# windingwind/seal-3d

Hardware: AMD Instinct MI355X
Metric: train samples/s (NGP -O step on synthetic Lego 800x800 rays) (higher is better)
Workload: dtype f16; 1 GPU; configs[1]: nerf_synthetic/lego-shaped NGP -O (hashgrid L16 F2 T2^19 + ffmlp 64x2/64x3 + raymarching), 800x800 cameras, 4096 rays/step/GPU; num_rays_per_gpu=4096, parallelism=ray-sharded dp1, pretrain_steps=384, launch=hip-graph replay

## Files before the change

### seal-3d_amd/csrc/raymarching.hip

```cpp
#include "s3d_common.hpp"
#include "s3d_step_tail.hpp"

namespace s3d {
namespace {

constexpr float kSqrt3 = 1.7320508075688772f;
constexpr float kRPi = 0.3183098861837907f;

__device__ __forceinline__ uint32_t expand_bits_any(uint32_t v) {
    v = (v * 0x00010001u) & 0xFF0000FFu;
    v = (v * 0x00000101u) & 0x0F00F00Fu;
    v = (v * 0x00000011u) & 0xC30C30C3u;
    v = (v * 0x00000005u) & 0x49249249u;
    return v;
}
__device__ __forceinline__ uint32_t expand_bits(uint32_t v) {
    v = (v | (v << 16)) & 0xFF0000FFu;
    v = (v | (v << 8)) & 0x0F00F00Fu;
    v = (v | (v << 4)) & 0xC30C30C3u;
    v = (v | (v << 2)) & 0x49249249u;
    return v;
}
__device__ __forceinline__ uint32_t morton3d(uint32_t x, uint32_t y, uint32_t z) {
    return expand_bits(x) | (expand_bits(y) << 1) | (expand_bits(z) << 2);
// ... 353 lines not shown
        const float s = sweep_sum_partials(partial + (size_t)c * stride, nblocks, wsum);
        total = c == 0 ? s : total + s;
    }
    if (threadIdx.x == 0) {
        const float mean = total * inv_n;
        record->mean = mean;
        record->thresh = density_thresh < mean ? density_thresh : mean;
        int32_t rows = *local_step;
        rows = rows < 0 ? 0 : (rows > 16 ? 16 : rows);
        int64_t count = 0;
        for (int32_t r = 0; r < rows; r++) count += step_ring[2 * r];
        record->count_lo = (uint32_t)((uint64_t)count & 0xFFFFFFFFull);
        record->count_hi = (uint32_t)((uint64_t)count >> 32);
        if (sweep_step) *sweep_step += 1;
    }
}

struct Ray {
    float ox, oy, oz, dx, dy, dz, rdx, rdy, rdz;
};
struct MarchParams {
    float bound, dt_gamma, dt_min, dt_max, rH, H3, Cf, Hf, Hm1, halfH;
    const uint8_t* grid;
};

__device__ __forceinline__ MarchParams make_params(float bound, float dt_gamma, uint32_t max_steps, uint32_t C,
                                                   uint32_t H, const uint8_t* grid) {
    MarchParams p;
    p.bound = bound; p.dt_gamma = dt_gamma;
    p.dt_min = 2 * kSqrt3 / (float)max_steps;
    p.dt_max = 2 * kSqrt3 * (float)(1 << (C - 1)) / (float)H;
    p.rH = 1 / (float)H;
    p.H3 = (float)(H * H * H);
    p.Cf = (float)C; p.Hf = (float)H; p.Hm1 = (float)(H - 1); p.halfH = 0.5f * (float)H;
    p.grid = grid;
    return p;
}

__device__ __forceinline__ Ray load_ray(const float* __restrict__ rays_o, const float* __restrict__ rays_d, uint32_t n) {
    Ray r;
    r.ox = rays_o[n * 3]; r.oy = rays_o[n * 3 + 1]; r.oz = rays_o[n * 3 + 2];
    r.dx = rays_d[n * 3]; r.dy = rays_d[n * 3 + 1]; r.dz = rays_d[n * 3 + 2];
    r.rdx = 1 / r.dx; r.rdy = 1 / r.dy; r.rdz = 1 / r.dz;
    return r;
}

__device__ __forceinline__ int mip_from_pos(float x, float y, float z, float Cf) {
    int e;
    (void)frexpf(fmaxf(fabsf(x), fmaxf(fabsf(y), fabsf(z))), &e);
    return (int)fminf(Cf - 1, fmaxf(0.0f, (float)e));
}
__device__ __forceinline__ int mip_from_dt(float dt, float Hf, float Cf) {
    int e;
    (void)frexpf((dt * Hf) * 0.5f, &e);
    return (int)fminf(Cf - 1, fmaxf(0.0f, (float)e));
}
__device__ __forceinline__ int mip_level(float x, float y, float z, float dt, const MarchParams& p) {
    const int la = mip_from_pos(x, y, z, p.Cf), lb = mip_from_dt(dt, p.Hf, p.Cf);
    return la > lb ? la : lb;
}

__global__ void k_mip_levels(const float* __restrict__ xyz, const float* __restrict__ dt, uint32_t N, float Hf, float Cf,
                             int32_t* __restrict__ mip_pos, int32_t* __restrict__ mip_dt) {
    for (uint32_t n = blockIdx.x * blockDim.x + threadIdx.x; n < N; n += gridDim.x * blockDim.x) {
        if (mip_pos) mip_pos[n] = mip_from_pos(xyz[n * 3], xyz[n * 3 + 1], xyz[n * 3 + 2], Cf);
        if (mip_dt) mip_dt[n] = mip_from_dt(dt[n], Hf, Cf);
    }
}

struct ProbeCell {
    float x, y, z, dt, mip_bound;
    int nx, ny, nz;
};
__device__ __forceinline__ uint32_t probe_cell(const Ray& r, const MarchParams& p, float t, ProbeCell& c) {
    c.x = clampf(__builtin_fmaf(t, r.dx, r.ox), -p.bound, p.bound);
    c.y = clampf(__builtin_fmaf(t, r.dy, r.oy), -p.bound, p.bound);
    c.z = clampf(__builtin_fmaf(t, r.dz, r.oz), -p.bound, p.bound);
    c.dt = clampf(t * p.dt_gamma, p.dt_min, p.dt_max);
    const int level = mip_level(c.x, c.y, c.z, c.dt, p);
    c.mip_bound = fminf(ldexpf(1.0f, level), p.bound);
    const float mip_rbound = 1 / c.mip_bound;
    c.nx = (int)clampf(__builtin_fmaf(c.x, mip_rbound, 1.0f) * p.halfH, 0.0f, p.Hm1);
    c.ny = (int)clampf(__builtin_fmaf(c.y, mip_rbound, 1.0f) * p.halfH, 0.0f, p.Hm1);
    c.nz = (int)clampf(__builtin_fmaf(c.z, mip_rbound, 1.0f) * p.halfH, 0.0f, p.Hm1);
    return (uint32_t)((float)level * p.H3 + (float)morton3d((uint32_t)c.nx, (uint32_t)c.ny, (uint32_t)c.nz));
}
__device__ __forceinline__ float probe_exit(const Ray& r, const MarchParams& p, float t, const ProbeCell& c) {
    const float sx = copysignf(1.0f, r.dx), sy = copysignf(1.0f, r.dy), sz = copysignf(1.0f, r.dz);
    const float tx = __builtin_fmaf(__builtin_fmaf(__builtin_fmaf(0.5f, sx, (float)c.nx + 0.5f) * p.rH, 2.0f, -1.0f), c.mip_bound, -c.x) * r.rdx;
    const float ty = __builtin_fmaf(__builtin_fmaf(__builtin_fmaf(0.5f, sy, (float)c.ny + 0.5f) * p.rH, 2.0f, -1.0f), c.mip_bound, -c.y) * r.rdy;
    const float tz = __builtin_fmaf(__builtin_fmaf(__builtin_fmaf(0.5f, sz, (float)c.nz + 0.5f) * p.rH, 2.0f, -1.0f), c.mip_bound, -c.z) * r.rdz;
    return t + fmaxf(0.0f, fminf(tx, fminf(ty, tz)));
}
__device__ __forceinline__ bool probe(const Ray& r, const MarchParams& p, float t, float& x, float& y, float& z,
                                      float& dt, float& t_skip) {
    ProbeCell c;
    const uint32_t index = probe_cell(r, p, t, c);
    x = c.x; y = c.y; z = c.z; dt = c.dt;
    const bool occ = (p.grid[index >> 3] & (1u << (index & 7u))) != 0;
    if (!occ) t_skip = probe_exit(r, p, t, c);
    return occ;
}

__device__ __forceinline__ float skip_to(const MarchParams& p, float t, float tt) {
    do { t += clampf(t * p.dt_gamma, p.dt_min, p.dt_max); } while (t < tt);
    return t;
}

constexpr uint32_t kWsHeader = 4;

__global__ void __launch_bounds__(64) k_march_count(const float* __restrict__ rays_o, const float* __restrict__ rays_d,
                                                    const uint8_t* __restrict__ grid, float bound, float dt_gamma,
                                                    uint32_t max_steps, uint32_t N, uint32_t C, uint32_t H,
                                                    const float* __restrict__ nears, const float* __restrict__ fars,
                                                    const float* __restrict__ noises, int32_t* __restrict__ rays,
                                                    const int32_t* __restrict__ counter, uint32_t* __restrict__ ws) {
    const uint32_t n = blockIdx.x * 64 + threadIdx.x;
    uint32_t num_steps = 0;
    if (n < N) {
        const MarchParams p = make_params(bound, dt_gamma, max_steps, C, H, grid);
        const Ray r = load_ray(rays_o, rays_d, n);
        const float far = fars[n];
        float t = nears[n];
        t = __builtin_fmaf(clampf(t * dt_gamma, p.dt_min, p.dt_max), noises[n], t);
        while (t < far && num_steps < max_steps) {
            float x, y, z, dt, tt;
            if (probe(r, p, t, x, y, z, dt, tt)) { num_steps++; t += dt; }
            else t = skip_to(p, t, tt);
        }
    }
    const uint32_t incl = wave_incl_scan(num_steps);
    if (n < N) {
        rays[n * 3] = (int32_t)n;
        rays[n * 3 + 1] = (int32_t)(incl - num_steps);
        rays[n * 3 + 2] = (int32_t)num_steps;
    }
    if (threadIdx.x == 63) ws[kWsHeader + blockIdx.x] = incl;
    if (blockIdx.x == 0 && threadIdx.x == 0) ws[0] = (uint32_t)counter[0];
}

__global__ void __launch_bounds__(64) k_march_write(const float* __restrict__ rays_o, const float* __restrict__ rays_d,
                                                    const uint8_t* __restrict__ grid, float bound, float dt_gamma,
                                                    uint32_t max_steps, uint32_t N, uint32_t C, uint32_t H, uint32_t M,
                                                    const float* __restrict__ nears, const float* __restrict__ fars,
                                                    const float* __restrict__ noises, float* __restrict__ xyzs,
                                                    float* __restrict__ dirs, float* __restrict__ deltas,
                                                    int32_t* __restrict__ rays, int32_t* __restrict__ counter,
                                                    const uint32_t* __restrict__ ws) {
    uint32_t part = 0;
    for (uint32_t i = threadIdx.x; i < blockIdx.x; i += 64) part += ws[kWsHeader + i];
#pragma unroll
    for (int d = 32; d >= 1; d >>= 1) part += __shfl_xor(part, d, 64);
    const uint32_t base = ws[0] + part;
    if (blockIdx.x == gridDim.x - 1 && threadIdx.x == 0) {
        counter[0] = (int32_t)(base + ws[kWsHeader + blockIdx.x]);
        counter[1] = counter[1] + (int32_t)N;
    }
    const uint32_t n = blockIdx.x * 64 + threadIdx.x;
    if (n >= N) return;
    const uint32_t num_steps = (uint32_t)rays[n * 3 + 2];
    const uint32_t off = base + (uint32_t)rays[n * 3 + 1];
    rays[n * 3 + 1] = (int32_t)off;
    if (n == N - 1 && off + num_steps < M) zero_sample_rows(xyzs, dirs, deltas, off + num_steps, pad_end(off + num_steps, M), 0, 1);
    if (num_steps != 0 && off < M && off + num_steps > M) zero_sample_rows(xyzs, dirs, deltas, off, M, 0, 1);
    if (num_steps == 0 || off + num_steps > M) return;

    const MarchParams p = make_params(bound, dt_gamma, max_steps, C, H, grid);
    const Ray r = load_ray(rays_o, rays_d, n);
    const float far = fars[n];
    float t = nears[n];
    t = __builtin_fmaf(clampf(t * dt_gamma, p.dt_min, p.dt_max), noises[n], t);
    float last_t = t;
    float* px = xyzs + (size_t)off * 3;
    float* pd = dirs + (size_t)off * 3;
    float* pl = deltas + (size_t)off * 2;
    uint32_t step = 0;
    while (t < far && step < num_steps) {
        float x, y, z, dt, tt;
        if (probe(r, p, t, x, y, z, dt, tt)) {
            px[0] = x; px[1] = y; px[2] = z;
            pd[0] = r.dx; pd[1] = r.dy; pd[2] = r.dz;
            t += dt;
            pl[0] = dt; pl[1] = t - last_t;
            last_t = t;
            px += 3; pd += 3; pl += 2; step++;
        } else t = skip_to(p, t, tt);
    }
}


constexpr uint32_t kWin = 1024;
constexpr uint16_t kOcc = 0xFFFF;

template <bool CONST_DT, bool FAST>
__global__ void __launch_bounds__(64) __attribute__((amdgpu_waves_per_eu(4, 4))) k_march_count_wave(const float* __restrict__ rays_o, const float* __restrict__ rays_d,
                                                         const uint8_t* __restrict__ grid, float bound, float dt_gamma,
                                                         uint32_t max_steps, uint32_t N, uint32_t C, uint32_t H,
                                                         float* __restrict__ nears, float* __restrict__ fars,
                                                         float* __restrict__ noises, int32_t* __restrict__ rays,
                                                         const int32_t* __restrict__ counter, uint32_t* __restrict__ ws,
                                                         const float* __restrict__ aabb, float min_near,
                                                         const int32_t* __restrict__ noise_step, uint32_t noise_key) {
    __shared__ float T[kWin + 8];
    __shared__ uint16_t J[2][kWin + 2];
    __shared__ uint32_t mk[64];
    __shared__ uint32_t s_wn;
    __shared__ uint32_t lut[FAST ? 128 : 1];
    const uint32_t n = blockIdx.x, lane = threadIdx.x;
    if constexpr (FAST) {
        lut[lane] = expand_bits(lane);
        lut[lane + 64] = expand_bits(lane + 64);
    }
    const MarchParams p = make_params(bound, dt_gamma, max_steps, C, H, grid);
    const Ray r = load_ray(rays_o, rays_d, n);
    float far, t_carry, noise;
    if (aabb) {
        const float a[6] = {aabb[0], aabb[1], aabb[2], aabb[3], aabb[4], aabb[5]};
        near_far_of(rays_o, rays_d, n, a, min_near, t_carry, far);
        noise = noises ? (noise_step ? ray_noise(noise_key, (uint32_t)*noise_step, n) : noises[n]) : 0.0f;
        if (lane == 0) {
            nears[n] = t_carry;
            fars[n] = far;
            if (noises && noise_step) noises[n] = noise;
        }
    } else {
        far = fars[n];
        t_carry = nears[n];
        noise = noises[n];
    }
    const float dt0 = clampf(0.0f, p.dt_min, p.dt_max);
    auto dtf = [&](float t) { return CONST_DT ? dt0 : clampf(t * dt_gamma, p.dt_min, p.dt_max); };
    t_carry = __builtin_fmaf(clampf(t_carry * dt_gamma, p.dt_min, p.dt_max), noise, t_carry);
    float* tout = reinterpret_cast<float*>(ws + kWsHeader + N) + (size_t)n * max_steps;

    uint32_t num_steps = 0;
    float pending_tt = -INFINITY;
#ifdef S3D_MARCH_PROFILE
    long long tp[5] = {0, 0, 0, 0, 0};
    long long c0 = wall_clock64();
#define S3D_TICK(i) { const long long c1 = wall_clock64(); tp[i] += c1 - c0; c0 = c1; }
#else
#define S3D_TICK(i)
#endif
    for (;;) {
        if constexpr (CONST_DT) {
            float t = t_carry;
            uint32_t k = 0;
            const uint32_t bfar = __float_as_uint(far);
            while (k < kWin && t < far) {
                const float t1 = t + dt0, t2 = t1 + dt0;
                const uint32_t b0 = __float_as_uint(t), b1 = __float_as_uint(t1), b2 = __float_as_uint(t2);
                const uint32_t inc = b2 - b1;
                if (!(t > 0.0f) || (b0 >> 23) != (b2 >> 23) || (b0 >> 23) == 0 || inc == 0 || !(far > 0.0f) || bfar >= 0x7f800000u) {
                    if (lane == 0) T[k] = t;
                    k++;
                    t = t1;
                    continue;
                }
                const uint32_t hi = ((b1 >> 23) + 1) << 23;
                const uint32_t cnt = (hi - b1) / inc + 1;
                const uint32_t nfill = min(cnt, kWin - k);
                const uint32_t n_lt = bfar <= b1 ? 0u : min(cnt, (bfar - b1 + inc - 1) / inc);
                if (lane == 0) T[k] = t;
                for (uint32_t j = lane; j < nfill; j += 64) T[k + 1 + j] = __uint_as_float(b1 + j * inc);
                if (n_lt < nfill) {
                    k = k + 1 + n_lt;
                    t = __uint_as_float(b1 + n_lt * inc);
                    break;
                }
                k += nfill;
                t = __uint_as_float(b1 + (nfill - 1) * inc);
            }
            if (lane == 0) { T[k] = t; s_wn = k; }
        } else if (lane == 0) {
            float t = t_carry;
            uint32_t k = 0;
            while (k < kWin && t < far) {
                float v[8];
                v[0] = t;
#pragma unroll
                for (uint32_t i = 1; i < 8; i++) v[i] = v[i - 1] + dtf(v[i - 1]);
#pragma unroll
                for (uint32_t i = 0; i < 8; i++) T[k + i] = v[i];
                uint32_t c = 1;
#pragma unroll
                for (uint32_t i = 1; i < 8; i++) c += (v[i] < far) ? 1u : 0u;
                if (c < 8) {
                    float tn = v[1];
#pragma unroll
                    for (uint32_t i = 2; i < 8; i++) tn = (c == i) ? v[i] : tn;
                    k += c;
                    t = tn;
                    break;
                }
                k += 8;
                t = v[7] + dtf(v[7]);
            }
            T[k] = t;
            s_wn = k;
        }
        __syncthreads();
        S3D_TICK(0)
        const uint32_t wn = s_wn;
        uint32_t occm = 0;
        uint32_t headm = 0;
        auto skip_index = [&](uint32_t k, float tk, float tt) {
            const float t1 = T[k + 1];
            const float est = (tt - t1) / fmaxf(t1 - tk, 1e-30f);
            uint32_t m = k + 1 + (est > 0.0f ? (est < (float)kWin ? (uint32_t)est : kWin) : 0u);
            m = m < wn ? m : wn;
            while (m > k + 1 && !(T[m - 1] < tt)) m--;
            while (m < wn && T[m] < tt) m++;
            return (uint16_t)m;
        };
        if constexpr (FAST) {
            constexpr uint32_t kBatch = 8;
            const float mip_bound = fminf(1.0f, p.bound), mip_rbound = 1 / mip_bound;
            uint32_t prev_last = 0xffffffffu;
#pragma unroll 1
            for (uint32_t b0 = 0; b0 * 64 < wn; b0 += kBatch) {
                uint32_t bits[kBatch], idx[kBatch], cell[kBatch];
#pragma unroll
                for (uint32_t j = 0; j < kBatch; j++) {
                    const float t = T[lane + 64 * (b0 + j)];
                    const float x = clampf(__builtin_fmaf(t, r.dx, r.ox), -p.bound, p.bound);
                    const float y = clampf(__builtin_fmaf(t, r.dy, r.oy), -p.bound, p.bound);
                    const float z = clampf(__builtin_fmaf(t, r.dz, r.oz), -p.bound, p.bound);
                    const uint32_t nx = (uint32_t)(int)clampf(__builtin_fmaf(x, mip_rbound, 1.0f) * p.halfH, 0.0f, p.Hm1);
                    const uint32_t ny = (uint32_t)(int)clampf(__builtin_fmaf(y, mip_rbound, 1.0f) * p.halfH, 0.0f, p.Hm1);
                    const uint32_t nz = (uint32_t)(int)clampf(__builtin_fmaf(z, mip_rbound, 1.0f) * p.halfH, 0.0f, p.Hm1);
                    cell[j] = nx | (ny << 8) | (nz << 16);
                    idx[j] = (uint32_t)(float)(lut[nx] | (lut[ny] << 1) | (lut[nz] << 2));
                }
#pragma unroll
                for (uint32_t j = 0; j < kBatch; j++) bits[j] = (uint32_t)p.grid[idx[j] >> 3];
#pragma unroll
                for (uint32_t j = 0; j < kBatch; j++) {
                    const uint32_t i = b0 + j, k = lane + 64 * i;
                    uint32_t prev = (uint32_t)__builtin_amdgcn_update_dpp((int)cell[j], (int)cell[j], 0x138, 0xF, 0xF, false);
                    if (lane == 0) prev = prev_last;
                    prev_last = (uint32_t)__builtin_amdgcn_readlane((int)cell[j], 63);
                    if (cell[j] != prev) headm |= 1u << i;
                    if (k < wn) {
                        uint16_t e = (uint16_t)(k + 1);
                        if (bits[j] & (1u << (idx[j] & 7u))) {
                            occm |= 1u << i;
                        } else {
                            const float tk = T[k];
                            ProbeCell c;
                            c.x = clampf(__builtin_fmaf(tk, r.dx, r.ox), -p.bound, p.bound);
                            c.y = clampf(__builtin_fmaf(tk, r.dy, r.oy), -p.bound, p.bound);
                            c.z = clampf(__builtin_fmaf(tk, r.dz, r.oz), -p.bound, p.bound);
                            c.mip_bound = mip_bound;
                            c.nx = (int)(cell[j] & 255u); c.ny = (int)((cell[j] >> 8) & 255u); c.nz = (int)(cell[j] >> 16);
                            e = skip_index(k, tk, probe_exit(r, p, tk, c));
                        }
                        J[0][k] = e;
                    }
                }
            }
        } else {
            for (uint32_t k = lane; k < wn; k += 64) {
                float x, y, z, dt, tt;
                uint16_t e = (uint16_t)(k + 1);
                const float tk = T[k];
                if (!probe(r, p, tk, x, y, z, dt, tt)) e = skip_index(k, tk, tt);
                else occm |= 1u << (k >> 6);
                J[0][k] = e;
            }
        }
        S3D_TICK(1)
        if (lane == 0) J[0][wn] = (uint16_t)wn;
        mk[lane] = 0;
        uint32_t start = wn;
        for (uint32_t k = lane; k < wn; k += 64)
            if (!(T[k] < pending_tt)) { start = k; break; }
#pragma unroll
        for (int d = 32; d >= 1; d >>= 1) start = min(start, (uint32_t)__shfl_xor((int)start, d, 64));
        pending_tt = -INFINITY;
        __syncthreads();
        bool marked = false;
#ifdef S3D_MARCH_PROFILE
        uint32_t dbg_vm0 = 0;
#endif
        if constexpr (FAST) {
            uint32_t vm = 0;
#pragma unroll
            for (uint32_t i = 0; i < kWin / 64; i++) {
                const uint32_t k = lane + 64 * i;
                const bool in = k < wn && k >= start;
                if (in && ((((occm | headm) >> i) & 1u) || k == start)) vm |= 1u << i;
            }
            const uint32_t startbit = (start < wn && (start & 63u) == lane) ? (1u << (start >> 6)) : 0u;
#ifdef S3D_MARCH_PROFILE
            dbg_vm0 = vm;
#endif
            constexpr uint32_t kMaxPasses = 6;
            for (uint32_t pass = 0; pass < kMaxPasses && !marked; pass++) {
#pragma unroll
                for (uint32_t i = 0; i < kWin / 64; i++) {
                    if ((vm >> i) & 1u) {
                        const uint32_t tg = J[0][lane + 64 * i];
                        if (tg < wn) atomicOr(&mk[tg & 63], 1u << (tg >> 6));
                    }
                }
                __syncthreads();
                const uint32_t pm = mk[lane];
                const bool closed = __ballot((pm & ~vm) != 0u) == 0ull;
                const bool supported = __ballot((vm & ~startbit & ~pm) != 0u) == 0ull;
                marked = closed && supported;
                if (!marked) vm = closed ? (pm | startbit) : (vm | pm);
                __syncthreads();
                mk[lane] = marked ? vm : 0u;
                __syncthreads();
            }
        }
        if (!marked && lane == 0 && start < wn) mk[start & 63] = 1u << (start >> 6);
        __syncthreads();
        uint32_t cur = 0;
        constexpr uint32_t kPer = kWin / 64 + 1;
        const uint32_t iters = wn / 64 + 1;
        for (uint32_t span = 1; span < wn && !marked; span <<= 1) {
            const uint16_t* Jc = J[cur];
            uint16_t* Jn = J[cur ^ 1];
            uint32_t j1[kPer], j2[kPer];
            const uint32_t mw = mk[lane];
#pragma unroll
            for (uint32_t i = 0; i < kPer; i++)
                if (i < iters) { const uint32_t k = lane + 64 * i; j1[i] = k <= wn ? Jc[k] : wn; }
#pragma unroll
            for (uint32_t i = 0; i < kPer; i++)
                if (i < iters) j2[i] = Jc[j1[i]];
#pragma unroll
            for (uint32_t i = 0; i < kPer; i++)
                if (i < iters) {
                    const uint32_t k = lane + 64 * i;
                    if (((mw >> i) & 1u) && j1[i] < wn) atomicOr(&mk[j1[i] & 63], 1u << (j1[i] >> 6));
                    if (k <= wn) Jn[k] = (uint16_t)j2[i];
                }
            cur ^= 1;
            __syncthreads();
            if (start >= wn || J[cur][start] >= wn) break;
        }
        S3D_TICK(2)
#ifdef S3D_MARCH_PROFILE
        if (FAST && max_steps >= 256) {
            const uint32_t d = mk[lane] ^ dbg_vm0;
            uint32_t cnt = __popc(d), first = d ? (lane + 64u * (uint32_t)__builtin_ctz(d)) : 0xFFFFu;
#pragma unroll
            for (int s2 = 32; s2 >= 1; s2 >>= 1) { cnt += (uint32_t)__shfl_xor((int)cnt, s2, 64); first = min(first, (uint32_t)__shfl_xor((int)first, s2, 64)); }
            if (lane == 0) { tout[max_steps - 16] = (float)cnt; tout[max_steps - 15] = (float)first; tout[max_steps - 14] = (float)wn; tout[max_steps - 13] = (float)start; }
        }
#endif
        uint32_t last_empty = kWin;
        bool any_empty = false;
        for (uint32_t k0 = 0; k0 < wn && num_steps < max_steps; k0 += 64) {
            const uint32_t k = k0 + lane;
            const bool vis = k < wn && ((mk[lane] >> (k0 >> 6)) & 1u);
            const bool emit = vis && ((occm >> (k0 >> 6)) & 1u);
            if (vis && !emit) { last_empty = k; any_empty = true; }
            const unsigned long long m = __ballot(emit);
            const uint32_t rank = __builtin_amdgcn_mbcnt_hi((uint32_t)(m >> 32), __builtin_amdgcn_mbcnt_lo((uint32_t)m, 0u));
            if (emit && num_steps + rank < max_steps) tout[num_steps + rank] = T[k];
            num_steps = min(max_steps, num_steps + (uint32_t)__popcll(m));
        }
        uint32_t le = any_empty ? last_empty : 0u;
#pragma unroll
        for (int d = 32; d >= 1; d >>= 1) le = max(le, (uint32_t)__shfl_xor((int)le, d, 64));
        const bool had_empty = __ballot(any_empty) != 0;
        const bool more = (wn == kWin) && (num_steps < max_steps);
        if (more && had_empty) {
            float x, y, z, dt, tt;
            (void)probe(r, p, T[le], x, y, z, dt, tt);
            if (le + 1 >= wn || T[wn - 1] < tt) pending_tt = tt;
        }
        t_carry = T[kWin];
        __syncthreads();
        S3D_TICK(3)
        if (!more) break;
    }
#ifdef S3D_MARCH_PROFILE
    if (lane == 0 && max_steps >= 256) {
        for (int i = 0; i < 4; i++) tout[max_steps - 8 + i] = (float)tp[i];
    }
#endif
    if (lane == 0) {
        rays[n * 3] = (int32_t)n;
        rays[n * 3 + 2] = (int32_t)num_steps;
        ws[kWsHeader + n] = num_steps;
        if (n == 0) ws[0] = (uint32_t)counter[0];
    }
}

__global__ void __launch_bounds__(64) k_march_write_wave(const float* __restrict__ rays_o, const float* __restrict__ rays_d,
                                                         float bound, float dt_gamma, uint32_t max_steps, uint32_t N, uint32_t C,
                                                         uint32_t H, uint32_t M, const float* __restrict__ nears,
                                                         const float* __restrict__ noises, float* __restrict__ xyzs,
                                                         float* __restrict__ dirs, float* __restrict__ deltas,
                                                         int32_t* __restrict__ rays, int32_t* __restrict__ counter,
                                                         const uint32_t* __restrict__ ws) {
    const uint32_t n = blockIdx.x, lane = threadIdx.x;
    uint32_t part = 0;
    {
        const uint4* c4 = reinterpret_cast<const uint4*>(ws + kWsHeader);
        const uint32_t n4 = n / 4;
        uint32_t p0 = 0, p1 = 0, p2 = 0, p3 = 0;
        for (uint32_t i = lane; i < n4; i += 64) {
            const uint4 v = c4[i];
            p0 += v.x; p1 += v.y; p2 += v.z; p3 += v.w;
        }
        part = (p0 + p1) + (p2 + p3);
        const uint32_t r0 = n4 * 4 + lane;
        if (r0 < n) part += ws[kWsHeader + r0];
    }
#pragma unroll
    for (int d = 32; d >= 1; d >>= 1) part += __shfl_xor(part, d, 64);
    const uint32_t off = ws[0] + part;
    const uint32_t num_steps = ws[kWsHeader + n];
    if (lane == 0) {
        rays[n * 3 + 1] = (int32_t)off;
        if (n == N - 1) { counter[0] = (int32_t)(off + num_steps); counter[1] = counter[1] + (int32_t)N; }
    }
    if (n == N - 1 && off + num_steps < M) zero_sample_rows(xyzs, dirs, deltas, off + num_steps, pad_end(off + num_steps, M), lane, 64);
    if (num_steps != 0 && off < M && off + num_steps > M) zero_sample_rows(xyzs, dirs, deltas, off, M, lane, 64);
    if (num_steps == 0 || off + num_steps > M) return;
    const MarchParams p = make_params(bound, dt_gamma, max_steps, C, H, nullptr);
    const Ray r = load_ray(rays_o, rays_d, n);
    float t0 = nears[n];
    t0 = __builtin_fmaf(clampf(t0 * dt_gamma, p.dt_min, p.dt_max), noises[n], t0);
    const float* tin = reinterpret_cast<const float*>(ws + kWsHeader + N) + (size_t)n * max_steps;
    for (uint32_t i = lane; i < num_steps; i += 64) {
        const float t = tin[i];
        float last_t = t0;
        if (i > 0) { const float tp = tin[i - 1]; last_t = tp + clampf(tp * dt_gamma, p.dt_min, p.dt_max); }
        const float dt = clampf(t * dt_gamma, p.dt_min, p.dt_max);
        const size_t o = (size_t)off + i;
        xyzs[o * 3] = clampf(__builtin_fmaf(t, r.dx, r.ox), -bound, bound);
        xyzs[o * 3 + 1] = clampf(__builtin_fmaf(t, r.dy, r.oy), -bound, bound);
        xyzs[o * 3 + 2] = clampf(__builtin_fmaf(t, r.dz, r.oz), -bound, bound);
        dirs[o * 3] = r.dx; dirs[o * 3 + 1] = r.dy; dirs[o * 3 + 2] = r.dz;
        deltas[o * 2] = dt;
        deltas[o * 2 + 1] = (t + dt) - last_t;
    }
}

constexpr uint32_t kWaveMarchMaxRays = 16384;

__global__ void __launch_bounds__(64) k_composite_train_fwd(const float* __restrict__ sigmas, const float* __restrict__ rgbs,
                                                            const float* __restrict__ deltas, const int32_t* __restrict__ rays,
                                                            uint32_t M, uint32_t N, float T_thresh,
                                                            float* __restrict__ weights_sum, float* __restrict__ depth,
                                                            float* __restrict__ image) {
    const uint32_t n = blockIdx.x * 64 + threadIdx.x;
    if (n >= N) return;
    const uint32_t index = (uint32_t)rays[n * 3], offset = (uint32_t)rays[n * 3 + 1], num_steps = (uint32_t)rays[n * 3 + 2];
    float r = 0, g = 0, b = 0, ws = 0, d = 0;
    if (num_steps != 0 && offset + num_steps <= M) {
        const float* s = sigmas + offset;
        const float* c = rgbs + (size_t)offset * 3;
        const float2* dl = reinterpret_cast<const float2*>(deltas) + offset;
        float T = 1.0f, t = 0;
        for (uint32_t step = 0; step < num_steps; step++) {
            const float2 dd = dl[step];
            const float alpha = 1.0f - __expf(-s[step] * dd.x);
            const float weight = alpha * T;
            r = __builtin_fmaf(weight, c[step * 3], r);
            g = __builtin_fmaf(weight, c[step * 3 + 1], g);
            b = __builtin_fmaf(weight, c[step * 3 + 2], b);
            t += dd.y;
            d = __builtin_fmaf(weight, t, d);
            ws += weight;
            T *= 1.0f - alpha;
            if (T < T_thresh) break;
        }
    }
    weights_sum[index] = ws; depth[index] = d;
    image[index * 3] = r; image[index * 3 + 1] = g; image[index * 3 + 2] = b;
}

__global__ void __launch_bounds__(64) k_composite_train_bwd(const float* __restrict__ grad_weights_sum,
                                                            const float* __restrict__ grad_image,
                                                            const float* __restrict__ sigmas, const float* __restrict__ rgbs,
                                                            const float* __restrict__ deltas, const int32_t* __restrict__ rays,
                                                            const float* __restrict__ weights_sum,
                                                            const float* __restrict__ image, uint32_t M, uint32_t N,
                                                            float T_thresh, float* __restrict__ grad_sigmas,
                                                            float* __restrict__ grad_rgbs) {
    const uint32_t n = blockIdx.x * 64 + threadIdx.x;
    if (n >= N) return;
    const uint32_t index = (uint32_t)rays[n * 3], offset = (uint32_t)rays[n * 3 + 1], num_steps = (uint32_t)rays[n * 3 + 2];
    if (n == N - 1 && offset + num_steps < M) zero_grad_rows(grad_sigmas, grad_rgbs, offset + num_steps, pad_end(offset + num_steps, M), 0, 1);
    if (num_steps != 0 && offset < M && offset + num_steps > M) zero_grad_rows(grad_sigmas, grad_rgbs, offset, M, 0, 1);
    if (num_steps == 0 || offset + num_steps > M) return;
    const float gws = grad_weights_sum[index];
    const float gi0 = grad_image[index * 3], gi1 = grad_image[index * 3 + 1], gi2 = grad_image[index * 3 + 2];
    const float r_final = image[index * 3], g_final = image[index * 3 + 1], b_final = image[index * 3 + 2];
    const float ws_final = weights_sum[index];
    const float* s = sigmas + offset;
    const float* c = rgbs + (size_t)offset * 3;
    const float2* dl = reinterpret_cast<const float2*>(deltas) + offset;
    float* gs = grad_sigmas + offset;
    float* gc = grad_rgbs + (size_t)offset * 3;
    float T = 1.0f, r = 0, g = 0, b = 0, ws = 0;
    for (uint32_t step = 0; step < num_steps; step++) {
        const float2 dd = dl[step];
        const float c0 = c[step * 3], c1 = c[step * 3 + 1], c2 = c[step * 3 + 2];
        const float alpha = 1.0f - __expf(-s[step] * dd.x);
        const float weight = alpha * T;
        r = __builtin_fmaf(weight, c0, r); g = __builtin_fmaf(weight, c1, g); b = __builtin_fmaf(weight, c2, b);
        ws += weight;
        T *= 1.0f - alpha;
        gc[step * 3] = gi0 * weight; gc[step * 3 + 1] = gi1 * weight; gc[step * 3 + 2] = gi2 * weight;
        float acc = gi0 * __builtin_fmaf(T, c0, -(r_final - r));
        acc = __builtin_fmaf(gi1, __builtin_fmaf(T, c1, -(g_final - g)), acc);
        acc = __builtin_fmaf(gi2, __builtin_fmaf(T, c2, -(b_final - b)), acc);
        acc = __builtin_fmaf(gws, 1 - ws_final, acc);
        gs[step] = dd.x * acc;
        if (T < T_thresh) {
            zero_grad_rows(grad_sigmas, grad_rgbs, offset + step + 1, offset + num_steps, 0, 1);
            break;
        }
    }
}


__device__ __forceinline__ float wave_scan_mul(float v, uint32_t lane) {
#pragma unroll
    for (int d = 1; d < 64; d <<= 1) { const float o = __shfl_up(v, d, 64); if (lane >= (uint32_t)d) v *= o; }
    return v;
}
__device__ __forceinline__ float wave_scan_add(float v, uint32_t lane) {
#pragma unroll
    for (int d = 1; d < 64; d <<= 1) { const float o = __shfl_up(v, d, 64); if (lane >= (uint32_t)d) v += o; }
    return v;
}
__device__ __forceinline__ float wave_sum(float v) {
#pragma unroll
    for (int d = 32; d >= 1; d >>= 1) v += __shfl_xor(v, d, 64);
    return v;
}

struct RayPixel { float r, g, b, ws, depth; };
__device__ __forceinline__ RayPixel composite_ray_fwd_wave(const float* __restrict__ sigmas, const float* __restrict__ rgbs,
                                                          const float* __restrict__ deltas, uint32_t offset, uint32_t num_steps,
                                                          uint32_t M, float T_thresh, uint32_t lane) {
    float r = 0, g = 0, b = 0, ws = 0, dsum = 0;
    if (num_steps != 0 && offset + num_steps <= M) {
        float T_carry = 1.0f, t_carry = 0.0f;
        for (uint32_t base = 0; base < num_steps; base += 64) {
            const uint32_t i = base + lane;
            const bool valid = i < num_steps;
            const size_t o = (size_t)offset + i;
            const float sg = valid ? sigmas[o] : 0.0f;
            const float2 dd = valid ? reinterpret_cast<const float2*>(deltas)[o] : make_float2(0.0f, 0.0f);
            const float c0 = valid ? rgbs[o * 3] : 0.0f, c1 = valid ? rgbs[o * 3 + 1] : 0.0f, c2 = valid ? rgbs[o * 3 + 2] : 0.0f;
            const float alpha = 1.0f - __expf(-sg * dd.x);
            const float P = wave_scan_mul(1.0f - alpha, lane);
            float Pex = __shfl_up(P, 1, 64);
            if (lane == 0) Pex = 1.0f;
            const float T = T_carry * Pex;
            const float tc = t_carry + wave_scan_add(dd.y, lane);
            const bool used = valid && (i == 0 || !(T < T_thresh));
            const float w = used ? alpha * T : 0.0f;
            r += w * c0; g += w * c1; b += w * c2; ws += w; dsum += w * tc;
            T_carry *= __shfl(P, 63, 64);
            t_carry = __shfl(tc, 63, 64);
            if (T_carry < T_thresh) break;
        }
        r = wave_sum(r); g = wave_sum(g); b = wave_sum(b); ws = wave_sum(ws); dsum = wave_sum(dsum);
    }
    return RayPixel{r, g, b, ws, dsum};
}

__global__ void __launch_bounds__(256) k_composite_train_fwd_wave(const float* __restrict__ sigmas, const float* __restrict__ rgbs,
                                                                 const float* __restrict__ deltas, const int32_t* __restrict__ rays,
                                                                 uint32_t M, uint32_t N, float T_thresh,
                                                                 float* __restrict__ weights_sum, float* __restrict__ depth,
                                                                 float* __restrict__ image) {
    const uint32_t lane = threadIdx.x & 63;
    const uint32_t n = blockIdx.x * 4 + (threadIdx.x >> 6);
    if (n >= N) return;
    const uint32_t index = (uint32_t)rays[n * 3], offset = (uint32_t)rays[n * 3 + 1], num_steps = (uint32_t)rays[n * 3 + 2];
    const RayPixel px = composite_ray_fwd_wave(sigmas, rgbs, deltas, offset, num_steps, M, T_thresh, lane);
    if (lane == 0) {
        weights_sum[index] = px.ws; depth[index] = px.depth;
        image[index * 3] = px.r; image[index * 3 + 1] = px.g; image[index * 3 + 2] = px.b;
    }
}

__device__ __forceinline__ void composite_ray_bwd_wave(const float* __restrict__ sigmas, const float* __restrict__ rgbs,
                                                       const float* __restrict__ deltas, uint32_t n, uint32_t offset,
                                                       uint32_t num_steps, uint32_t M, uint32_t N, float T_thresh, float gws,
                                                       float gi0, float gi1, float gi2, float rf, float gf, float bf, float wsf,
                                                       float* __restrict__ grad_sigmas, float* __restrict__ grad_rgbs,
                                                       uint32_t lane) {
    if (n == N - 1 && offset + num_steps < M) zero_grad_rows(grad_sigmas, grad_rgbs, offset + num_steps, pad_end(offset + num_steps, M), lane, 64);
    if (num_steps != 0 && offset < M && offset + num_steps > M) zero_grad_rows(grad_sigmas, grad_rgbs, offset, M, lane, 64);
    if (num_steps == 0 || offset + num_steps > M) return;
    float T_carry = 1.0f, rc = 0, gc = 0, bc = 0;
    for (uint32_t base = 0; base < num_steps; base += 64) {
        const uint32_t i = base + lane;
        const bool valid = i < num_steps;
        const size_t o = (size_t)offset + i;
        const float sg = valid ? sigmas[o] : 0.0f;
        const float d0 = valid ? deltas[o * 2] : 0.0f;
        const float c0 = valid ? rgbs[o * 3] : 0.0f, c1 = valid ? rgbs[o * 3 + 1] : 0.0f, c2 = valid ? rgbs[o * 3 + 2] : 0.0f;
        const float alpha = 1.0f - __expf(-sg * d0);
        const float P = wave_scan_mul(1.0f - alpha, lane);
        float Pex = __shfl_up(P, 1, 64);
        if (lane == 0) Pex = 1.0f;
        const float T = T_carry * Pex;
        const float Tn = T_carry * P;
        const bool used = valid && (i == 0 || !(T < T_thresh));
        const float w = used ? alpha * T : 0.0f;
        const float rr = rc + wave_scan_add(w * c0, lane), gg = gc + wave_scan_add(w * c1, lane), bb = bc + wave_scan_add(w * c2, lane);
        if (used) {
            grad_rgbs[o * 3] = gi0 * w; grad_rgbs[o * 3 + 1] = gi1 * w; grad_rgbs[o * 3 + 2] = gi2 * w;
// ... 794 lines not shown
```

Baseline: 689.9 million samples/s.

## Compute empty-cell skip targets lazily and compact them for load balance

Empty-cell skip targets (probe_exit plus skip_index) are no longer computed eagerly for every unoccupied sample. The kernel now builds a ballot-compacted list of only the empty samples that head a cell or start the window, and processes that list with all lanes working densely. Further targets are computed on demand during the marking passes, and all remaining ones are filled in if marking fails. This cuts the divergent, expensive probe work per window, at the cost of an extra compaction pass, extra syncs, and more complex control flow.

```diff
diff --git a/seal-3d_amd/csrc/raymarching.hip b/seal-3d_amd/csrc/raymarching.hip
--- a/seal-3d_amd/csrc/raymarching.hip
+++ b/seal-3d_amd/csrc/raymarching.hip
@@ -679,8 +679,14 @@
         __syncthreads();
         S3D_TICK(0)
         const uint32_t wn = s_wn;
+        uint32_t start = wn;
+        for (uint32_t k = lane; k < wn; k += 64)
+            if (!(T[k] < pending_tt)) { start = k; break; }
+#pragma unroll
+        for (int d = 32; d >= 1; d >>= 1) start = min(start, (uint32_t)__shfl_xor((int)start, d, 64));
         uint32_t occm = 0;
         uint32_t headm = 0;
+        uint32_t skipm = 0;
         auto skip_index = [&](uint32_t k, float tk, float tt) {
             const float t1 = T[k + 1];
             const float est = (tt - t1) / fmaxf(t1 - tk, 1e-30f);
@@ -689,6 +695,19 @@
             while (m > k + 1 && !(T[m - 1] < tt)) m--;
             while (m < wn && T[m] < tt) m++;
             return (uint16_t)m;
+        };
+        auto skip_of = [&](uint32_t k) {
+            const float mip_bound = fminf(1.0f, p.bound), mip_rbound = 1 / mip_bound;
+            const float tk = T[k];
+            ProbeCell c;
+            c.x = clampf(__builtin_fmaf(tk, r.dx, r.ox), -p.bound, p.bound);
+            c.y = clampf(__builtin_fmaf(tk, r.dy, r.oy), -p.bound, p.bound);
+            c.z = clampf(__builtin_fmaf(tk, r.dz, r.oz), -p.bound, p.bound);
+            c.mip_bound = mip_bound;
+            c.nx = (int)(uint32_t)(int)clampf(__builtin_fmaf(c.x, mip_rbound, 1.0f) * p.halfH, 0.0f, p.Hm1);
+            c.ny = (int)(uint32_t)(int)clampf(__builtin_fmaf(c.y, mip_rbound, 1.0f) * p.halfH, 0.0f, p.Hm1);
+            c.nz = (int)(uint32_t)(int)clampf(__builtin_fmaf(c.z, mip_rbound, 1.0f) * p.halfH, 0.0f, p.Hm1);
+            return skip_index(k, tk, probe_exit(r, p, tk, c));
         };
         if constexpr (FAST) {
             constexpr uint32_t kBatch = 8;
@@ -718,23 +737,29 @@
                     if (lane == 0) prev = prev_last;
                     prev_last = (uint32_t)__builtin_amdgcn_readlane((int)cell[j], 63);
                     if (cell[j] != prev) headm |= 1u << i;
-                    if (k < wn) {
-                        uint16_t e = (uint16_t)(k + 1);
-                        if (bits[j] & (1u << (idx[j] & 7u))) {
-                            occm |= 1u << i;
-                        } else {
-                            const float tk = T[k];
-                            ProbeCell c;
-                            c.x = clampf(__builtin_fmaf(tk, r.dx, r.ox), -p.bound, p.bound);
-                            c.y = clampf(__builtin_fmaf(tk, r.dy, r.oy), -p.bound, p.bound);
-                            c.z = clampf(__builtin_fmaf(tk, r.dz, r.oz), -p.bound, p.bound);
-                            c.mip_bound = mip_bound;
-                            c.nx = (int)(cell[j] & 255u); c.ny = (int)((cell[j] >> 8) & 255u); c.nz = (int)(cell[j] >> 16);
-                            e = skip_index(k, tk, probe_exit(r, p, tk, c));
-                        }
-                        J[0][k] = e;
+                    if (k < wn && (bits[j] & (1u << (idx[j] & 7u)))) {
+                        occm |= 1u << i;
+                        J[0][k] = (uint16_t)(k + 1);
                     }
                 }
+            }
+            uint16_t* list = J[1];
+            uint32_t nlist = 0;
+#pragma unroll
+            for (uint32_t i = 0; i < kWin / 64; i++) {
+                const uint32_t k = lane + 64 * i;
+                const bool want = k < wn && k >= start && !((occm >> i) & 1u) && (((headm >> i) & 1u) || k == start);
+                const unsigned long long m = __ballot(want);
+                if (want) {
+                    list[nlist + __builtin_amdgcn_mbcnt_hi((uint32_t)(m >> 32), __builtin_amdgcn_mbcnt_lo((uint32_t)m, 0u))] = (uint16_t)k;
+                    skipm |= 1u << i;
+                }
+                nlist += (uint32_t)__popcll(m);
+            }
+            __syncthreads();
+            for (uint32_t q = lane; q < nlist; q += 64) {
+                const uint32_t k = list[q];
+                J[0][k] = skip_of(k);
             }
         } else {
             for (uint32_t k = lane; k < wn; k += 64) {
@@ -749,11 +774,6 @@
         S3D_TICK(1)
         if (lane == 0) J[0][wn] = (uint16_t)wn;
         mk[lane] = 0;
-        uint32_t start = wn;
-        for (uint32_t k = lane; k < wn; k += 64)
-            if (!(T[k] < pending_tt)) { start = k; break; }
-#pragma unroll
-        for (int d = 32; d >= 1; d >>= 1) start = min(start, (uint32_t)__shfl_xor((int)start, d, 64));
         pending_tt = -INFINITY;
         __syncthreads();
         bool marked = false;
@@ -786,10 +806,26 @@
                 const bool closed = __ballot((pm & ~vm) != 0u) == 0ull;
                 const bool supported = __ballot((vm & ~startbit & ~pm) != 0u) == 0ull;
                 marked = closed && supported;
-                if (!marked) vm = closed ? (pm | startbit) : (vm | pm);
+                if (!marked) {
+                    vm = closed ? (pm | startbit) : (vm | pm);
+                    for (uint32_t todo = vm & ~occm & ~skipm; todo; todo &= todo - 1u) {
+                        const uint32_t k = lane + 64 * (uint32_t)__builtin_ctz(todo);
+                        J[0][k] = skip_of(k);
+                    }
+                    skipm |= vm & ~occm;
+                }
                 __syncthreads();
                 mk[lane] = marked ? vm : 0u;
                 __syncthreads();
+            }
+        }
+        if constexpr (FAST) {
+            if (!marked) {
+#pragma unroll 1
+                for (uint32_t i = 0; i < kWin / 64; i++) {
+                    const uint32_t k = lane + 64 * i;
+                    if (k < wn && !(((occm | skipm) >> i) & 1u)) J[0][k] = skip_of(k);
+                }
             }
         }
         if (!marked && lane == 0 && start < wn) mk[start & 63] = 1u << (start >> 6);
```

New measurement: 695.5 million samples/s (median of 4 runs). Within noise of the previous version (+0.8%).
